# annalam/seqkit

Measured on AMD Instinct MI355X. Metric: M reads/s demultiplex (150bp, 96 barcodes) at 1/8 GPUs; % HBM roofline, higher is better.
Workload: dtype u8

## Files before the change

### seqkit_amd/csrc/sk_census.hip

```cpp
#include <hip/hip_runtime.h>

#include <algorithm>
#include <cstdlib>
#include <cstring>
#include <vector>

#include "sk_internal.h"

namespace sk {

typedef unsigned long long u64;
typedef uint32_t u32;

struct CensusSlot {
	u64 klo;
	u64 khi_inv;
	u64 count;
	u64 first_inv;
};

constexpr int kSpillBucketsLog2 = 8;
constexpr int kSpillBuckets = 1 << kSpillBucketsLog2;
__device__ __forceinline__ uint32_t census_bucket(uint32_t h) { return h >> (32 - kSpillBucketsLog2); }
constexpr int kSpillMaxLen = 24;
constexpr int kSpillMaxGrid = 1024;

struct CensusSpill {
	uint4 *key = nullptr;
	u32 *hist = nullptr;
	u32 *btot = nullptr;
	u32 *wg_count = nullptr;
	u32 *wg_stats = nullptr;
	u32 *work = nullptr;
	u32 cap = 0;
	u32 direct_above = 0;
	u32 grid = 0;
	u32 merge_copies = 0;
};

constexpr int kRecRowBits = 25;
__device__ __forceinline__ u32 census_rec_row(u32 w) { return w & ((1u << kRecRowBits) - 1u); }
__device__ __forceinline__ u32 census_rec_count(u32 w) { return (((w >> 27) & 31u) + 1u) << (5u * ((w >> kRecRowBits) & 3u)); }

struct Census {
	CensusSpill sp;
	size_t sp_records = 0;
	int sp_grid = 0;
	CensusSlot *tab = nullptr;
	u64 slots = 0;
	u32 *log = nullptr;
	u32 *log_count = nullptr;
	u32 log_cap = 0;
	u64 *stats = nullptr;
	u64 distinct = 0;
	u64 *scratch = nullptr;
	size_t scratch_bytes = 0;
};

constexpr int kCensusStats = 4;
constexpr u64 kInitialSlots = 1ull << 26;
constexpr u32 kLogCap = 1u << 16;
constexpr int64_t kCensusChunk = 1 << 25;
constexpr int64_t kCensusMinChunk = 1 << 22;
constexpr int kLdsSlots = 2048;
constexpr int kLdsProbes = 8;
constexpr u32 kMaxProbes = 1u << 16;

struct LdsTable {
	u64 klo[kLdsSlots];
	u64 khi_inv[kLdsSlots];
	u64 first_inv[kLdsSlots];
	u32 count[kLdsSlots];
};

__device__ __forceinline__ u32 census_hash(u64 klo, u64 khi)
{
	const u32 w0 = (u32)klo, w1 = (u32)(klo >> 32), w2 = (u32)khi, w3 = (u32)(khi >> 32);
	u32 h = w0 * 0x9E3779B1u ^ __builtin_rotateleft32(w1, 13) * 0x85EBCA77u ^ w2 * 0xC2B2AE3Du ^ __builtin_rotateleft32(w3, 7) * 0x27D4EB2Fu;
	h ^= h >> 15;
	h *= 0x2C1B3C6Du;
	h ^= h >> 12;
	h *= 0x297A2D39u;
	h ^= h >> 15;
	return h;
}

constexpr u32 kClassLo = 0x412B4300u;
constexpr u32 kClassHi = 0xFF54474Eu;
__device__ __forceinline__ u32 census_classify(u32 x, u32 &diff)
{
	const u32 lower = x & (x >> 1) & 0x20202020u;
	const u32 y = x ^ lower;
	const u32 sel = (y ^ (y >> 5)) & 0x07070707u;
	diff = y ^ __builtin_amdgcn_perm(kClassHi, kClassLo, sel);
	return sel | (lower >> 2);
}
static const char kCensusAlphabet[17] = "\0C+ANGT??c?angt?";

struct SlotView { u64 k, v; };

__device__ __forceinline__ SlotView census_peek(const CensusSlot *s)
{
	typedef u32 u32x4_t __attribute__((ext_vector_type(4)));
	u32x4_t w;
	asm volatile("global_load_dwordx4 %0, %1, off sc1" : "=&v"(w) : "v"(s) : "memory");
	__builtin_amdgcn_s_waitcnt(0x0F70);
	asm volatile("" : "+v"(w));
	SlotView sv;
	sv.k = (u64)w[0] | ((u64)w[1] << 32);
	sv.v = (u64)w[2] | ((u64)w[3] << 32);
	return sv;
}

constexpr int kLogRegions = 256;
struct CensusTab {
	CensusSlot *tab;
	u64 mask;
	u32 sh;
	u32 *log;
	u32 *log_count;
	u32 log_cap;
};

__device__ __forceinline__ void census_log_claim(const CensusTab &t, const CensusSlot *s)
{
	if (t.log_cap == 0u) return;
	const u64 m = __ballot(1);
	const int leader = __ffsll((unsigned long long)m) - 1;
	const u32 rank = __builtin_amdgcn_mbcnt_hi((u32)(m >> 32), __builtin_amdgcn_mbcnt_lo((u32)m, 0u));
// ... 694 lines not shown
		counted += __shfl_xor(counted, o);
		rejected += __shfl_xor(rejected, o);
		overflow += __shfl_xor(overflow, o);
	}
	__syncthreads();
	u32 *wg_stats = front;
	if (tid < kCensusStats) wg_stats[tid] = 0u;
	__syncthreads();
	if (lane == 0) {
		if (claimed) atomicAdd(&wg_stats[0], claimed);
		if (counted) atomicAdd(&wg_stats[1], counted);
		if (rejected) atomicAdd(&wg_stats[2], rejected);
		if (overflow) atomicAdd(&wg_stats[3], overflow);
	}
	__syncthreads();
	if (SPILL) { if (tid < kCensusStats) a.sp.wg_stats[blockIdx.x * kCensusStats + tid] = wg_stats[tid]; }
	else if (tid < kCensusStats && wg_stats[tid] != 0u) atomicAdd(&a.stats[tid], (u64)wg_stats[tid]);
#ifdef SK_CENSUS_STAMPS
	SK_STAMP(9);
	if (lane == 0 && blockIdx.x * nwave + wave < 8192)
		for (int i = 0; i < kStampSlots; i++) g_census_stamps[(blockIdx.x * nwave + wave) * kStampSlots + i] = st_acc[i];
#endif
}

__device__ __forceinline__ u32 census_block_exclusive(u32 mine, u32 *ws, u32 *total)
{
	const int lane = threadIdx.x & 63, wave = threadIdx.x >> 6, nw = (blockDim.x + 63) >> 6;
	u32 v = mine;
#pragma unroll
	for (int o = 1; o < 64; o <<= 1) {
		const u32 t = __shfl_up(v, o);
		if (lane >= o) v += t;
	}
	__syncthreads();
	if (lane == 63) ws[wave] = v;
	__syncthreads();
	if (wave == 0) {
		const u32 w = lane < nw ? ws[lane] : 0u;
		u32 x = w;
#pragma unroll
		for (int o = 1; o < 16; o <<= 1) {
			const u32 t = __shfl_up(x, o);
			if (lane >= o) x += t;
		}
		if (lane < nw) ws[lane] = x - w;
		if (lane == nw - 1) ws[16] = x;
	}
	__syncthreads();
	if (total) *total = ws[16];
	return v - mine + ws[wave];
}

__device__ __forceinline__ u32 census_spill_total(const CensusSpill &sp, u32 *red)
{
	u32 v = 0u;
	for (u32 g = threadIdx.x; g < sp.grid; g += blockDim.x) v += sp.wg_count[g];
	for (int o = 32; o > 0; o >>= 1) v += __shfl_xor(v, o);
	if ((threadIdx.x & 63) == 0) red[threadIdx.x >> 6] = v;
	__syncthreads();
	u32 tot = 0u;
	for (u32 w = 0; w < (blockDim.x + 63) / 64; w++) tot += red[w];
	__syncthreads();
	return tot;
}

__device__ __forceinline__ void census_add_stats(u64 *stats, u32 claimed, u32 overflow, u32 *red)
{
	for (int o = 32; o > 0; o >>= 1) {
		claimed += __shfl_xor(claimed, o);
		overflow += __shfl_xor(overflow, o);
	}
	__syncthreads();
	if (threadIdx.x < 2) red[threadIdx.x] = 0u;
	__syncthreads();
	if ((threadIdx.x & 63) == 0) {
		if (claimed) atomicAdd(&red[0], claimed);
		if (overflow) atomicAdd(&red[1], overflow);
	}
	__syncthreads();
	if (threadIdx.x == 0 && red[0] != 0u) atomicAdd(&stats[0], (u64)red[0]);
	if (threadIdx.x == 1 && red[1] != 0u) atomicAdd(&stats[3], (u64)red[1]);
}

constexpr int kCombineThreads = 512;
#ifndef SK_COMBINE_CHUNK
#define SK_COMBINE_CHUNK 16384
#endif
constexpr int kCombineChunk = SK_COMBINE_CHUNK;
__global__ __launch_bounds__(kCombineThreads, 4) void census_combine_kernel(const CensusArgs a)
{
	__shared__ LdsTable lt_s;
	__shared__ u32 cpre[kSpillBuckets + 1];
	__shared__ u32 gpre[kSpillMaxGrid + 1];
	__shared__ u32 red[kCombineThreads / 64];
	__shared__ u32 ws[17];
	__shared__ u32 item_s, nlist;
	__shared__ uint16_t list[kLdsSlots];
	LdsTable *lt = &lt_s;
	const int tid = threadIdx.x;
	const u32 grid = a.sp.grid;
#ifdef SK_CENSUS_STAMPS
	u64 cst_acc[kStampSlots] = {};
	u64 cst_last = __builtin_amdgcn_s_memtime();
#endif
	if (blockIdx.x == 0) {
		__shared__ u32 ssum[kCensusStats];
		if (tid < kCensusStats) ssum[tid] = 0u;
		__syncthreads();
		u32 v = 0u;
		for (u32 i = tid; i < grid * kCensusStats; i += blockDim.x) v += a.sp.wg_stats[i];
		for (int o = 32; o >= kCensusStats; o >>= 1) v += __shfl_xor(v, o);
		if ((tid & 63) < kCensusStats && v != 0u) atomicAdd(&ssum[tid & 3], v);
		__syncthreads();
		if (tid < kCensusStats && ssum[tid] != 0u) atomicAdd(&a.stats[tid], (u64)ssum[tid]);
	}
	if (census_spill_total(a.sp, red) > a.sp.direct_above) return;
	{
		static_assert(kSpillBuckets <= kCombineThreads, "one bucket per thread");
		const u32 c = tid < kSpillBuckets ? (a.sp.btot[tid] + kCombineChunk - 1) / kCombineChunk : 0u;
		u32 total;
		const u32 before = census_block_exclusive(c, ws, &total);
		if (tid < kSpillBuckets) cpre[tid] = before;
		if (tid == 0) cpre[kSpillBuckets] = total;
		__syncthreads();
	}
	const u32 items = cpre[kSpillBuckets];
	SK_CSTAMP(0);
	u32 claimed = 0, overflow = 0;
	int b_have = -1;
	for (;;) {
		__syncthreads();
		if (tid == 0) item_s = atomicAdd(a.sp.work, 1u);
		for (int i = tid; i < (int)(sizeof(LdsTable) / 8); i += blockDim.x) reinterpret_cast<u64 *>(lt)[i] = 0ull;
		__syncthreads();
		const u32 item = item_s;
		SK_CSTAMP(1);
		if (item >= items) break;
		int b = 0;
		for (int o = kSpillBuckets / 2; o > 0; o >>= 1) if (cpre[b + o] <= item) b += o;
		if (b != b_have) {
			u32 carry = 0u;
			for (u32 g0 = 0; g0 < grid; g0 += blockDim.x) {
				const u32 g = g0 + tid;
				const u32 v = g < grid ? a.sp.hist[(size_t)b * grid + g] : 0u;
				u32 total;
				const u32 before = census_block_exclusive(v, ws, &total);
				if (g < grid) gpre[g] = carry + before;
				carry += total;
			}
			if (tid == 0) gpre[grid] = carry;
			__syncthreads();
			b_have = b;
		}
		const u32 lo = (item - cpre[b]) * kCombineChunk;
		const u32 hi = min(gpre[grid], lo + kCombineChunk);
		u32 gcur = 0u;
		{
			const u32 i = lo + tid;
			u32 l = 0u, r = grid;
			while (r - l > 1u) { const u32 m = (l + r) >> 1; if (gpre[m] <= i) l = m; else r = m; }
			gcur = l;
		}
		SK_CSTAMP(2);
		const uint4 *const base = a.sp.key + (size_t)b * a.sp.cap;
		const size_t gpitch = (size_t)kSpillBuckets * a.sp.cap;
		constexpr int kAhead = 4;
		uint4 kk[kAhead], kn[kAhead];
		auto fetch = [&](u32 i0, uint4 (&dst)[kAhead]) {
#pragma unroll
			for (int q = 0; q < kAhead; q++) {
				const u32 i = i0 + (u32)q * blockDim.x;
				if (i < hi) {
					while (gpre[gcur + 1] <= i) gcur++;
					dst[q] = base[(size_t)gcur * gpitch + (i - gpre[gcur])];
				} else dst[q] = make_uint4(0u, 0u, 0u, 0u);
			}
		};
		fetch(lo + tid, kk);
		for (u32 i0 = lo + tid; i0 < hi; i0 += kAhead * blockDim.x) {
			fetch(i0 + kAhead * blockDim.x, kn);
			bool dir[kAhead], have[kAhead];
			u64 klo[kAhead], khi[kAhead], first_inv[kAhead];
			u32 cnt[kAhead], hh[kAhead];
#pragma unroll
			for (int q = 0; q < kAhead; q++) {
				const uint4 k = kk[q];
				have[q] = i0 + (u32)q * blockDim.x < hi;
				klo[q] = 0xF0000000ull | ((u64)k.x << 32);
				khi[q] = (u64)k.y | ((u64)k.z << 32);
				first_inv[q] = ~(u64)(a.row_base + census_rec_row(k.w));
				cnt[q] = census_rec_count(k.w);
				hh[q] = census_hash(klo[q], khi[q]);
			}
			SK_CSTAMP(3);
			lds_count_many<kAhead>(lt, have, hh, klo, khi, cnt, first_inv, dir);
			SK_CSTAMP(4);
			bool any_dir = false;
#pragma unroll
			for (int q = 0; q < kAhead; q++) any_dir = any_dir || dir[q];
			if (__any(any_dir)) census_insert_many<kAhead>(a.t, dir, klo, khi, cnt, first_inv, claimed, overflow);
			SK_CSTAMP(5);
#pragma unroll
			for (int q = 0; q < kAhead; q++) kk[q] = kn[q];
		}
		__syncthreads();
		SK_CSTAMP(6);
		if (tid == 0) nlist = 0u;
		__syncthreads();
		for (int i = tid; i < kLdsSlots; i += blockDim.x)
			if (lt->klo[i] != 0) list[atomicAdd(&nlist, 1u)] = (uint16_t)i;
		__syncthreads();
		for (u32 j0 = tid; j0 < nlist; j0 += kAhead * blockDim.x) {
			bool want[kAhead];
			u64 klo[kAhead], khi[kAhead], first_inv[kAhead];
			u32 cnt[kAhead];
#pragma unroll
			for (int q = 0; q < kAhead; q++) {
				const u32 j = j0 + (u32)q * blockDim.x;
				want[q] = j < nlist;
				const int i = list[want[q] ? j : 0u];
				klo[q] = lt->klo[i]; khi[q] = ~lt->khi_inv[i]; first_inv[q] = lt->first_inv[i]; cnt[q] = lt->count[i];
			}
			census_insert_many<kAhead>(a.t, want, klo, khi, cnt, first_inv, claimed, overflow);
		}
		SK_CSTAMP(7);
	}
	census_add_stats(a.stats, claimed, overflow, red);
#ifdef SK_CENSUS_STAMPS
	SK_CSTAMP(8);
	if ((tid & 63) == 0 && blockIdx.x * (kCombineThreads / 64) + (tid >> 6) < 8192)
		for (int i = 0; i < kStampSlots; i++) g_combine_stamps[(blockIdx.x * (kCombineThreads / 64) + (tid >> 6)) * kStampSlots + i] = cst_acc[i];
#endif
}

constexpr int kDirectThreads = 512;
__global__ __launch_bounds__(kDirectThreads) void census_direct_kernel(const CensusArgs a, const int split)
{
	__shared__ u32 red[16];
	const bool mine = census_spill_total(a.sp, red) > a.sp.direct_above;
	if (blockIdx.x == 0) {
		if (threadIdx.x < (u32)kSpillBuckets) a.sp.btot[threadIdx.x] = 0u;
		if (threadIdx.x == 0) *a.sp.work = 0u;
	}
	if (!mine) return;
	const u32 g = blockIdx.x / (u32)split, part = blockIdx.x % (u32)split;
	u32 claimed = 0, overflow = 0;
	__shared__ u32 bpre[kSpillBuckets + 1];
	__shared__ u32 ws[17];
	{
		static_assert(kSpillBuckets <= kDirectThreads, "one bucket per thread");
		const u32 v = threadIdx.x < (u32)kSpillBuckets ? a.sp.hist[(size_t)threadIdx.x * a.sp.grid + g] : 0u;
		u32 total;
		const u32 before = census_block_exclusive(v, ws, &total);
		if (threadIdx.x < (u32)kSpillBuckets) bpre[threadIdx.x] = before;
		if (threadIdx.x == 0) bpre[kSpillBuckets] = total;
		__syncthreads();
	}
	const u32 n = bpre[kSpillBuckets];
	const u32 rot = n != 0u ? (u32)(((u64)g * 0x9E3779B1ull) % n) : 0u;
	const uint4 *const key = a.sp.key + (size_t)g * kSpillBuckets * a.sp.cap;
	for (u32 jj = part * blockDim.x + threadIdx.x; jj < n; jj += (u32)split * blockDim.x) {
		u32 j = jj + rot;
		j = j >= n ? j - n : j;
		u32 l = 0u, r = (u32)kSpillBuckets;
		while (r - l > 1u) { const u32 m = (l + r) >> 1; if (bpre[m] <= j) l = m; else r = m; }
		const uint4 k = key[(size_t)l * a.sp.cap + (j - bpre[l])];
		const u64 klo = 0xF0000000ull | ((u64)k.x << 32), khi = (u64)k.y | ((u64)k.z << 32);
		const u32 c = census_rec_count(k.w);
		if (!census_insert(a.t, klo, khi, (u64)c, ~(u64)(a.row_base + census_rec_row(k.w)), claimed)) overflow += c;
	}
	census_add_stats(a.stats, claimed, overflow, red);
}

__global__ __launch_bounds__(256) void census_rehash_kernel(const CensusSlot *old_tab, u64 old_slots, const CensusTab t, u64 *stats)
{
	u32 claimed = 0, overflow = 0;
	for (u64 i = (u64)blockIdx.x * blockDim.x + threadIdx.x; i < old_slots; i += (u64)gridDim.x * blockDim.x) {
		const CensusSlot s = old_tab[i];
		if (s.klo == 0) continue;
		if (!census_insert(t, s.klo, ~s.khi_inv, s.count, s.first_inv, claimed)) overflow++;
	}
	if (overflow) atomicAdd(&stats[3], (u64)overflow);
}

__global__ __launch_bounds__(256) void census_hist_kernel(const CensusSlot *tab, u64 slots, u64 *hist)
{
	__shared__ u32 lh[64];
	if (threadIdx.x < 64) lh[threadIdx.x] = 0;
	__syncthreads();
	for (u64 i = (u64)blockIdx.x * blockDim.x + threadIdx.x; i < slots; i += (u64)gridDim.x * blockDim.x) {
		const u64 klo = tab[i].klo, c = tab[i].count;
		if (klo != 0 && c != 0) atomicAdd(&lh[63 - __clzll(c)], 1u);
	}
	__syncthreads();
	if (threadIdx.x < 64 && lh[threadIdx.x]) atomicAdd(&hist[threadIdx.x], (u64)lh[threadIdx.x]);
}

__global__ __launch_bounds__(256) void census_compact_kernel(const CensusSlot *tab, u64 slots, u64 min_count, u64 *out, u64 cap)
{
	for (u64 i = (u64)blockIdx.x * blockDim.x + threadIdx.x; i < slots; i += (u64)gridDim.x * blockDim.x) {
		const CensusSlot s = tab[i];
		if (s.klo != 0 && s.count >= min_count && s.count != 0) {
			const u64 at = atomicAdd(&out[0], 1ull);
			if (at < cap) {
				u64 *e = out + 4 + at * 4;
				e[0] = s.klo; e[1] = s.khi_inv; e[2] = s.count; e[3] = s.first_inv;
			}
		}
	}
}

constexpr int kCensusVariants = kCensusMaxSub * 3 * 2;
static const void *census_variant(int v)
{
// ... 61 lines not shown
	while ((1ull << lg) < cs->slots) lg++;
	t.sh = (u32)(32 - lg);
	t.log = cs->log;
	t.log_count = cs->log_count;
	t.log_cap = cs->log_cap;
	return t;
}

__global__ __launch_bounds__(256) void census_clear_kernel(const CensusTab t)
{
	__shared__ u32 cnt[kLogRegions];
	__shared__ u32 over;
	if (threadIdx.x == 0) over = 0u;
	__syncthreads();
	for (int r = threadIdx.x; r < kLogRegions; r += blockDim.x) {
		const u32 c = t.log_count[r * 32];
		cnt[r] = c < t.log_cap ? c : t.log_cap;
		if (c > t.log_cap || t.log_cap == 0u) over = 1u;
	}
	__syncthreads();
	uint4 *const p = reinterpret_cast<uint4 *>(t.tab);
	if (over) {
		const u64 n = (t.mask + 1) * (sizeof(CensusSlot) / 16);
		for (u64 i = (u64)blockIdx.x * blockDim.x + threadIdx.x; i < n; i += (u64)gridDim.x * blockDim.x) p[i] = make_uint4(0u, 0u, 0u, 0u);
		return;
	}
	const int r = blockIdx.x & (kLogRegions - 1);
	const u32 per = gridDim.x / kLogRegions ? gridDim.x / kLogRegions : 1u, part = blockIdx.x / kLogRegions;
	for (u32 i = part * blockDim.x + threadIdx.x; i < cnt[r]; i += per * blockDim.x) {
		const u64 slot = t.log[(size_t)r * t.log_cap + i];
		p[2 * slot] = make_uint4(0u, 0u, 0u, 0u);
		p[2 * slot + 1] = make_uint4(0u, 0u, 0u, 0u);
	}
}

hipError_t census_reset(Census *cs, int n_cu, hipStream_t st)
{
	hipError_t e = hipMemsetAsync(cs->stats, 0, kCensusStats * sizeof(u64), st);
	if (e == hipSuccess) {
		census_clear_kernel<<<kLogRegions * 8, 256, 0, st>>>(census_tab_of(cs));
		e = hipGetLastError();
	}
	if (e == hipSuccess) e = hipMemsetAsync(cs->log_count, 0, (size_t)kLogRegions * 32 * sizeof(u32), st);
	(void)n_cu;
	cs->distinct = 0;
	return e;
}

hipError_t census_stats(Census *cs, uint64_t out[4], hipStream_t st)
{
	u64 h[kCensusStats];
	hipError_t e = hipMemcpyAsync(h, cs->stats, sizeof h, hipMemcpyDeviceToHost, st);
	if (e == hipSuccess) e = hipStreamSynchronize(st);
	if (e != hipSuccess) return e;
	cs->distinct = h[0];
	for (int i = 0; i < kCensusStats; i++) out[i] = h[i];
	return hipSuccess;
}

uint64_t census_slots(const Census *cs) { return cs->slots; }

static hipError_t census_reserve(Census *cs, u64 incoming, int n_cu, hipStream_t st)
{
	const u64 need = 2 * (cs->distinct + incoming);
	if (need <= cs->slots) return hipSuccess;
	u64 slots = cs->slots;
	while (slots < need) slots <<= 1;
	if (slots > (1ull << 32)) return hipErrorOutOfMemory;
	CensusSlot *old_tab = cs->tab;
	const u64 old_slots = cs->slots;
	hipError_t e = census_alloc_table(cs, slots, st);
	if (e != hipSuccess) { (void)hipGetLastError(); cs->tab = old_tab; cs->slots = old_slots; return e; }
	e = hipMemsetAsync(cs->log_count, 0, (size_t)kLogRegions * 32 * sizeof(u32), st);
	if (e != hipSuccess) return e;
	census_rehash_kernel<<<n_cu * 8, 256, 0, st>>>(old_tab, old_slots, census_tab_of(cs), cs->stats);
	e = hipGetLastError();
	if (e == hipSuccess) e = hipStreamSynchronize(st);
	(void)hipFree(old_tab);
	return e;
}

static void census_spill_free(Census *cs)
{
	void *ptrs[] = {cs->sp.key, cs->sp.hist, cs->sp.btot, cs->sp.wg_count, cs->sp.wg_stats, cs->sp.work};
	for (void *q : ptrs) if (q) (void)hipFree(q);
	cs->sp = CensusSpill();
	cs->sp_records = 0;
	cs->sp_grid = 0;
}

static hipError_t census_spill_reserve(Census *cs, int grid, u32 cap, hipStream_t st)
{
	const size_t records = (size_t)grid * kSpillBuckets * cap;
	if (records <= cs->sp_records && grid <= cs->sp_grid) return hipSuccess;
	const size_t want_records = std::max(records, cs->sp_records);
	const int want_grid = std::max(grid, cs->sp_grid);
	hipError_t e = hipStreamSynchronize(st);
	if (e != hipSuccess) return e;
	census_spill_free(cs);
	e = hipMalloc((void **)&cs->sp.key, want_records * sizeof(uint4));
	if (e == hipSuccess) e = hipMalloc((void **)&cs->sp.hist, (size_t)want_grid * kSpillBuckets * sizeof(u32));
	if (e == hipSuccess) e = hipMalloc((void **)&cs->sp.btot, kSpillBuckets * sizeof(u32));
	if (e == hipSuccess) e = hipMalloc((void **)&cs->sp.wg_count, (size_t)want_grid * sizeof(u32));
	if (e == hipSuccess) e = hipMalloc((void **)&cs->sp.wg_stats, (size_t)want_grid * kCensusStats * sizeof(u32));
	if (e == hipSuccess) e = hipMalloc((void **)&cs->sp.work, sizeof(u32));
	if (e == hipSuccess) e = hipMemsetAsync(cs->sp.btot, 0, kSpillBuckets * sizeof(u32), st);
	if (e == hipSuccess) e = hipMemsetAsync(cs->sp.work, 0, sizeof(u32), st);
	if (e != hipSuccess) { (void)hipGetLastError(); census_spill_free(cs); return e; }
	cs->sp_records = want_records;
	cs->sp_grid = want_grid;
	return hipSuccess;
}

constexpr int64_t kSpillMinRows = 1 << 19;

hipError_t census_add(Census *cs, const uint8_t *bc, int bc_stride, int L, int64_t n, const int32_t *assign, int64_t row_base,
                      int n_cu, hipStream_t st)
{
	if (bc_stride > kCensusMaxStride) return hipErrorInvalidValue;
	int R = kCensusStepBytes / (64 * bc_stride);
	R = R < 1 ? 1 : (R > kCensusMaxSub ? kCensusMaxSub : R);
	if (const char *ev = getenv("SK_CENSUS_TILES")) { const int v = atoi(ev); if (v >= 1 && v <= R) R = v; }
	const int nw_dwords = L <= 8 ? 2 : (L <= 20 ? 5 : 8);
	auto slot_bytes = [&](int r, bool spill_layout) {
		const int queue_cap = 64 + r * 64;
		int bytes = queue_cap * (4 * nw_dwords + 4);
		if (!spill_layout) {
			const int flush_end = ((queue_cap * 4 + 64 * 4 * nw_dwords + 15) & ~15) + kCensusQueue * 20;
			if (bytes < flush_end) bytes = flush_end;
		}
		return (bytes + 15) & ~15;
	};
	const int nw_class = L <= 8 ? 0 : (L <= 20 ? 1 : 2);
	const int front_entry_bytes = nw_class == 2 ? 52 : 36;
	auto plan_lds = [&](int r, bool spill_layout, int &tile_slot, int &front_entries) {
		tile_slot = slot_bytes(r, spill_layout);
		size_t lds = (size_t)kCensusWaves * tile_slot + 64 + (kSpillBuckets + 4) * sizeof(u32);
		front_entries = (int)((160 * 1024 - 16 - lds) / front_entry_bytes) & ~63;
		if (const char *ev = getenv("SK_CENSUS_FRONT_ENTRIES")) { const int v = atoi(ev) & ~63; if (v >= 64 && v <= front_entries) front_entries = v; }
		return lds + (((size_t)front_entries * front_entry_bytes + 15) & ~(size_t)15);
	};
	int wgs_per_cu = 1;
	if (const char *ev = getenv("SK_CENSUS_WGS")) { const int v = atoi(ev); if (v >= 1 && v <= 4) wgs_per_cu = v; }
	int direct_pct = 50;
	if (const char *ev = getenv("SK_CENSUS_SPILL_MAX_PCT")) { const int v = atoi(ev); if (v >= 0 && v <= 100) direct_pct = v; }
	int64_t spill_min_rows = kSpillMinRows;
	if (const char *ev = getenv("SK_CENSUS_SPILL_MIN_ROWS_LOG2")) { const int lg = atoi(ev); if (lg >= 6 && lg <= 30) spill_min_rows = (int64_t)1 << lg; }
	int direct_split = 8;
	if (const char *ev = getenv("SK_CENSUS_DIRECT_SPLIT")) { const int v = atoi(ev); if (v >= 1 && v <= 64) direct_split = v; }
	int merge_copies = 1;
	if (const char *ev = getenv("SK_CENSUS_MERGE_RECORDS")) merge_copies = atoi(ev) != 0;
	int spill_mode = -1;
	if (const char *ev = getenv("SK_CENSUS_SPILL")) spill_mode = atoi(ev) != 0;
	int64_t chunk = kCensusChunk, min_chunk = kCensusMinChunk;
	if (const char *ev = getenv("SK_CENSUS_CHUNK_LOG2")) { const int lg = atoi(ev); if (lg >= 6 && lg <= kRecRowBits) chunk = (int64_t)1 << lg; }
	if (const char *ev = getenv("SK_CENSUS_MIN_CHUNK_LOG2")) { const int lg = atoi(ev); if (lg >= 6 && lg <= 30) min_chunk = (int64_t)1 << lg; }
	{
		const int64_t max_rows = ((((int64_t)1 << 31) - (1 << 24)) / bc_stride) & ~(int64_t)63;
		if (chunk > max_rows) chunk = max_rows;
	}
	if (min_chunk > chunk) min_chunk = chunk;
	int64_t nr = 0;
	for (int64_t o = 0; o < n; o += nr) {
		nr = (n - o) < chunk ? (n - o) : chunk;
		hipError_t e = hipSuccess;
		if (2 * (cs->distinct + (u64)nr) > cs->slots && !getenv("SK_CENSUS_TRUST_SLOTS")) {
			uint64_t s[4];
			e = census_stats(cs, s, st);
			if (e != hipSuccess) return e;
			const int64_t room = (int64_t)(cs->slots / 2) - (int64_t)cs->distinct;
			const int64_t least = nr < min_chunk ? nr : min_chunk;
			if (room >= least) nr = nr < room ? nr : room;
			else e = census_reserve(cs, (u64)nr, n_cu, st);
			if (e != hipSuccess) return e;
			if (nr < n - o && nr >= 64) nr &= ~(int64_t)63;
		}
		cs->distinct += (u64)nr;
		CensusArgs a;
		a.bc = bc + o * (int64_t)bc_stride;
		a.bc_stride = bc_stride;
		a.L = L;
		a.n = nr;
		a.assign = assign ? assign + o : nullptr;
		a.row_base = row_base + o;
		a.t = census_tab_of(cs);
		a.stats = cs->stats;
		a.long_way_only = getenv("SK_CENSUS_LONG_WAY_ONLY") && atoi(getenv("SK_CENSUS_LONG_WAY_ONLY")) != 0;
		bool spill = L <= kSpillMaxLen && (spill_mode < 0 ? nr >= spill_min_rows : spill_mode != 0);
		const int Rk = (spill && nw_class >= 1 && !getenv("SK_CENSUS_TILES")) ? 1 : R;
		auto grid_of = [&](int r) {
			const int64_t groups = (nr + (int64_t)64 * r * kCensusWaves - 1) / ((int64_t)64 * r * kCensusWaves);
			const int g = n_cu * wgs_per_cu;
			return g > groups ? (int)groups : g;
		};
		int grid = grid_of(Rk);
		a.sp = CensusSpill();
		if (spill) {
			const int64_t nsteps = (nr + (int64_t)64 * Rk - 1) / ((int64_t)64 * Rk);
			const int64_t per_wave = (nsteps + (int64_t)grid * kCensusWaves - 1) / ((int64_t)grid * kCensusWaves);
			const int64_t wg_rows = per_wave * kCensusWaves * Rk * 64;
			const int64_t cap = (((wg_rows + kSpillBuckets - 1) / kSpillBuckets) * 2 + 256 + 7) & ~(int64_t)7;
			e = (grid <= kSpillMaxGrid && cap * kSpillBuckets < ((int64_t)1 << 27)) ? census_spill_reserve(cs, grid, (u32)cap, st) : hipErrorInvalidValue;
			if (e != hipSuccess) { (void)hipGetLastError(); spill = false; grid = grid_of(Rk); }
			else {
				a.sp = cs->sp;
				a.sp.cap = (u32)cap;
				a.sp.grid = (u32)grid;
				a.sp.direct_above = (u32)((uint64_t)nr * (uint64_t)direct_pct / 100);
				a.sp.merge_copies = (u32)merge_copies;
			}
		}
		int tile_slot = 0, front_entries = 0;
		const size_t lds = plan_lds(Rk, spill, tile_slot, front_entries);
		hipLaunchKernelGGL(reinterpret_cast<void (*)(const CensusArgs, const int, const int)>(const_cast<void *>(census_variant(((Rk - 1) * 3 + nw_class) * 2 + (spill ? 1 : 0)))),
		                   dim3(grid), dim3(kCensusWaves * 64), lds, st, a, tile_slot, front_entries);
		if (spill) {
			census_combine_kernel<<<2 * n_cu, kCombineThreads, 0, st>>>(a);
			census_direct_kernel<<<grid * direct_split, kDirectThreads, 0, st>>>(a, direct_split);
		}
		e = hipGetLastError();
		if (e != hipSuccess) return e;
	}
	return hipSuccess;
}

static hipError_t census_scratch(Census *cs, size_t bytes)
{
	if (bytes <= cs->scratch_bytes) return hipSuccess;
	if (cs->scratch) { (void)hipFree(cs->scratch); cs->scratch = nullptr; cs->scratch_bytes = 0; }
	hipError_t e = hipMalloc((void **)&cs->scratch, bytes);
	if (e == hipSuccess) cs->scratch_bytes = bytes;
	return e;
}

hipError_t census_count_hist(Census *cs, uint64_t hist[64], int n_cu, hipStream_t st)
{
	hipError_t e = census_scratch(cs, 64 * sizeof(u64));
	if (e == hipSuccess) e = hipMemsetAsync(cs->scratch, 0, 64 * sizeof(u64), st);
	if (e != hipSuccess) return e;
	census_hist_kernel<<<n_cu * 8, 256, 0, st>>>(cs->tab, cs->slots, cs->scratch);
	e = hipGetLastError();
	if (e == hipSuccess) e = hipMemcpyAsync(hist, cs->scratch, 64 * sizeof(u64), hipMemcpyDeviceToHost, st);
	if (e == hipSuccess) e = hipStreamSynchronize(st);
	return e;
}

hipError_t census_entries(Census *cs, uint64_t min_count, CensusEntry *out, uint64_t cap, uint64_t *total, int n_cu, hipStream_t st)
{
	uint64_t s[4];
	hipError_t e = census_stats(cs, s, st);
	if (e != hipSuccess) return e;
	const u64 room = std::min<u64>(cap, s[0]);
	e = census_scratch(cs, (4 + room * 4) * sizeof(u64));
	if (e == hipSuccess) e = hipMemsetAsync(cs->scratch, 0, 4 * sizeof(u64), st);
	if (e != hipSuccess) return e;
	census_compact_kernel<<<n_cu * 8, 256, 0, st>>>(cs->tab, cs->slots, min_count ? min_count : 1, cs->scratch, room);
	e = hipGetLastError();
	if (e != hipSuccess) return e;
	u64 found = 0;
	e = hipMemcpyAsync(&found, cs->scratch, sizeof found, hipMemcpyDeviceToHost, st);
	if (e == hipSuccess) e = hipStreamSynchronize(st);
	if (e != hipSuccess) return e;
	*total = found;
	const u64 got = std::min<u64>(found, room);
	std::vector<u64> raw(got * 4);
	if (got) {
		e = hipMemcpy(raw.data(), cs->scratch + 4, got * 4 * sizeof(u64), hipMemcpyDeviceToHost);
		if (e != hipSuccess) return e;
	}
	std::vector<u64> order(got);
	for (u64 i = 0; i < got; i++) order[i] = i;
	std::sort(order.begin(), order.end(), [&](u64 x, u64 y) { return raw[x * 4 + 3] > raw[y * 4 + 3]; });
	for (u64 i = 0; i < got; i++) {
		const u64 *r = &raw[order[i] * 4];
		const u64 klo = r[0], khi = ~r[1];
		const u32 kw[4] = {(u32)(klo >> 32), (u32)khi, (u32)(khi >> 32), (u32)klo};
		CensusEntry &en = out[i];
		memset(en.barcode, 0, sizeof en.barcode);
		for (int j = 0; j < 31; j++) {
			const int q = j >> 2, b = j & 3;
			const u32 c = (kw[q >> 1] >> (8 * b + 4 * (q & 1))) & 15u;
			if (c == 0) break;
			en.barcode[j] = kCensusAlphabet[c];
		}
		en.count = r[2];
		en.first_row = (int64_t)~r[3];
	}
	return hipSuccess;
}

}

#ifdef SK_CENSUS_STAMPS
extern "C" int sk_debug_census_stamps(unsigned long long *out, int waves)
{
	return (int)hipMemcpyFromSymbol(out, HIP_SYMBOL(sk::g_census_stamps), (size_t)waves * sk::kStampSlots * sizeof(unsigned long long));
}
extern "C" int sk_debug_combine_stamps(unsigned long long *out, int waves)
{
// ... 4 lines not shown
```

Before: 6767.

## Sub-partition large spill buckets by hash before combine for LDS locality

Adds two passes, subcount and subscatter, that split each large spill bucket into up to 512 hash sub-buckets and scatter the records into a contiguous sub-key buffer. The combine kernel then handles each sub-bucket range as one work item, so each workgroup's LDS table sees a narrower key range and fewer keys fall through to direct global-table inserts. Work items are also claimed in batches of four to reduce contention on the shared work counter. The cost is two extra kernel launches, an extra read and write of the spilled records, and a larger scratch allocation.

```diff
diff --git a/seqkit_amd/csrc/sk_census.hip b/seqkit_amd/csrc/sk_census.hip
--- a/seqkit_amd/csrc/sk_census.hip
+++ b/seqkit_amd/csrc/sk_census.hip
@@ -36,7 +36,17 @@
 	u32 direct_above = 0;
 	u32 grid = 0;
 	u32 merge_copies = 0;
+	uint4 *skey = nullptr;
+	u32 *subcnt = nullptr;
+	u32 *subcur = nullptr;
+	u32 *subpre = nullptr;
+	u32 *subitems = nullptr;
+	u32 sub_cap = 0;
+	u32 sub_above = 0;
+	u32 sub_split = 0;
 };
+constexpr int kSubMaxLog2 = 9;
+constexpr int kSubMax = 1 << kSubMaxLog2;
 
 constexpr int kRecRowBits = 25;
 __device__ __forceinline__ u32 census_rec_row(u32 w) { return w & ((1u << kRecRowBits) - 1u); }
@@ -45,6 +55,7 @@
 struct Census {
 	CensusSpill sp;
 	size_t sp_records = 0;
+	size_t sp_sub_records = 0;
 	int sp_grid = 0;
 	CensusSlot *tab = nullptr;
 	u64 slots = 0;
@@ -905,7 +916,210 @@
 	if (threadIdx.x == 1 && red[1] != 0u) atomicAdd(&stats[3], (u64)red[1]);
 }
 
+constexpr u32 kSubTarget = 1024;
+constexpr u32 kSubAbove = 4096;
+constexpr u32 kSubSplit = 4096;
 constexpr int kCombineThreads = 512;
+constexpr int kPartAhead = 4;
+constexpr u32 kPartChunk = kPartAhead * kCombineThreads;
+
+__device__ __forceinline__ int census_sub_log2(const CensusSpill &sp, u32 n)
+{
+	if (n <= sp.sub_above) return 0;
+	const u32 target = min(kSubTarget, max(sp.sub_above, 1u));
+	const u32 want = (n + target - 1u) / target;
+	const int lg = 32 - __clz((int)(want - 1u));
+	return lg > kSubMaxLog2 ? kSubMaxLog2 : lg;
+}
+__device__ __forceinline__ u32 census_sub_of(u32 h, int lg) { return (h >> (32 - kSpillBucketsLog2 - lg)) & ((1u << lg) - 1u); }
+__device__ __forceinline__ u32 census_rec_hash(const uint4 k) { return census_hash(0xF0000000ull | ((u64)k.x << 32), (u64)k.y | ((u64)k.z << 32)); }
+
+__device__ __forceinline__ void census_scan_regions(const CensusSpill &sp, int b, u32 *gpre, u32 *ws)
+{
+	const u32 grid = sp.grid;
+	u32 carry = 0u;
+	for (u32 g0 = 0; g0 < grid; g0 += blockDim.x) {
+		const u32 g = g0 + threadIdx.x;
+		const u32 v = g < grid ? sp.hist[(size_t)b * grid + g] : 0u;
+		u32 total;
+		const u32 before = census_block_exclusive(v, ws, &total);
+		if (g < grid) gpre[g] = carry + before;
+		carry += total;
+	}
+	if (threadIdx.x == 0) gpre[grid] = carry;
+	__syncthreads();
+}
+__device__ __forceinline__ u32 census_region_of(const u32 *gpre, u32 grid, u32 i)
+{
+	u32 l = 0u, r = grid;
+	while (r - l > 1u) { const u32 m = (l + r) >> 1; if (gpre[m] <= i) l = m; else r = m; }
+	return l;
+}
+__device__ __forceinline__ uint4 census_region_record(const CensusSpill &sp, int b, const u32 *gpre, u32 &gcur, u32 i)
+{
+	while (gpre[gcur + 1] <= i) gcur++;
+	return sp.key[(size_t)b * sp.cap + (size_t)gcur * kSpillBuckets * sp.cap + (i - gpre[gcur])];
+}
+
+__device__ __forceinline__ bool census_part_plan(const CensusSpill &sp, u32 *cpre, u32 *bbase, uint8_t *blg, u32 *red, u32 *ws)
+{
+	static_assert(kSpillBuckets <= kCombineThreads, "one bucket per thread");
+	if (census_spill_total(sp, red) > sp.direct_above) return false;
+	const int tid = threadIdx.x;
+	const u32 bt = tid < kSpillBuckets ? sp.btot[tid] : 0u;
+	const int lg = tid < kSpillBuckets ? census_sub_log2(sp, bt) : 0;
+	u32 total;
+	u32 before = census_block_exclusive(lg ? (bt + kPartChunk - 1u) / kPartChunk : 0u, ws, &total);
+	if (tid < kSpillBuckets) { cpre[tid] = before; blg[tid] = (uint8_t)lg; }
+	if (tid == 0) cpre[kSpillBuckets] = total;
+	if (bbase) {
+		before = census_block_exclusive(lg ? bt : 0u, ws, nullptr);
+		if (tid < kSpillBuckets) bbase[tid] = before;
+	}
+	__syncthreads();
+	return cpre[kSpillBuckets] != 0u;
+}
+
+#ifdef SK_CENSUS_STAMPS
+#define SK_PART_STAMPS_BEGIN u64 cst_acc[kStampSlots] = {}; u64 cst_last = __builtin_amdgcn_s_memtime()
+#define SK_PART_STAMPS_END(first, n) do { if ((threadIdx.x & 63) == 0 && blockIdx.x * (kCombineThreads / 64) + (threadIdx.x >> 6) < 8192) \
+		for (int i_ = (first); i_ < (first) + (n); i_++) g_combine_stamps[(blockIdx.x * (kCombineThreads / 64) + (threadIdx.x >> 6)) * kStampSlots + i_] = cst_acc[i_]; } while (0)
+#else
+#define SK_PART_STAMPS_BEGIN do { } while (0)
+#define SK_PART_STAMPS_END(first, n) do { } while (0)
+#endif
+
+__global__ __launch_bounds__(kCombineThreads) void census_subcount_kernel(const CensusArgs a)
+{
+	__shared__ u32 cpre[kSpillBuckets + 1];
+	__shared__ u32 gpre[kSpillMaxGrid + 1];
+	__shared__ u32 cnt[kSubMax];
+	__shared__ u32 red[kCombineThreads / 64];
+	__shared__ u32 ws[17];
+	__shared__ uint8_t blg[kSpillBuckets];
+	const int tid = threadIdx.x;
+	SK_PART_STAMPS_BEGIN;
+	if (!census_part_plan(a.sp, cpre, nullptr, blg, red, ws)) { SK_PART_STAMPS_END(9, 2); return; }
+	const u32 chunks = cpre[kSpillBuckets];
+	const u32 c0 = (u32)((u64)blockIdx.x * chunks / gridDim.x), c1 = (u32)((u64)(blockIdx.x + 1u) * chunks / gridDim.x);
+	SK_CSTAMP(9);
+	int b_have = -1, lg = 0;
+	auto flush = [&]() {
+		__syncthreads();
+		if (b_have >= 0)
+			for (u32 s = tid; s < (1u << lg); s += blockDim.x)
+				if (cnt[s] != 0u) atomicAdd(&a.sp.subcnt[(size_t)b_have * kSubMax + s], cnt[s]);
+		__syncthreads();
+	};
+	for (u32 c = c0; c < c1; c++) {
+		int b = 0;
+		for (int o = kSpillBuckets / 2; o > 0; o >>= 1) if (cpre[b + o] <= c) b += o;
+		if (b != b_have) {
+			flush();
+			census_scan_regions(a.sp, b, gpre, ws);
+			lg = blg[b];
+			for (u32 s = tid; s < (1u << lg); s += blockDim.x) cnt[s] = 0u;
+			__syncthreads();
+			b_have = b;
+		}
+		const u32 lo = (c - cpre[b]) * kPartChunk;
+		const u32 hi = min(gpre[a.sp.grid], lo + kPartChunk);
+		u32 gcur = census_region_of(gpre, a.sp.grid, lo + tid);
+		uint4 k[kPartAhead];
+#pragma unroll
+		for (int q = 0; q < kPartAhead; q++) {
+			const u32 i = lo + tid + (u32)q * blockDim.x;
+			k[q] = i < hi ? census_region_record(a.sp, b, gpre, gcur, i) : make_uint4(0u, 0u, 0u, 0u);
+		}
+#pragma unroll
+		for (int q = 0; q < kPartAhead; q++)
+			if (lo + tid + (u32)q * blockDim.x < hi) atomicAdd(&cnt[census_sub_of(census_rec_hash(k[q]), lg)], 1u);
+	}
+	flush();
+	SK_CSTAMP(10);
+	SK_PART_STAMPS_END(9, 2);
+}
+
+__global__ __launch_bounds__(kCombineThreads) void census_subscatter_kernel(const CensusArgs a)
+{
+	__shared__ u32 cpre[kSpillBuckets + 1];
+	__shared__ u32 bbase[kSpillBuckets];
+	__shared__ u32 gpre[kSpillMaxGrid + 1];
+	__shared__ u32 cnt[kSubMax];
+	__shared__ u32 spre[kSubMax];
+	__shared__ u32 red[kCombineThreads / 64];
+	__shared__ u32 ws[17];
+	__shared__ uint8_t blg[kSpillBuckets];
+	static_assert(kSubMax <= kCombineThreads, "one sub-bucket per thread");
+	const int tid = threadIdx.x;
+	SK_PART_STAMPS_BEGIN;
+	if (!census_part_plan(a.sp, cpre, bbase, blg, red, ws)) { SK_PART_STAMPS_END(11, 4); return; }
+	const u32 chunks = cpre[kSpillBuckets];
+	const u32 split = max(a.sp.sub_split, 1u);
+	for (u32 b = blockIdx.x; b < (u32)kSpillBuckets; b += gridDim.x) {
+		const int lgb = blg[b];
+		if (lgb == 0) continue;
+		const u32 nsub = 1u << lgb;
+		const u32 v = (u32)tid < nsub ? a.sp.subcnt[(size_t)b * kSubMax + tid] : 0u;
+		u32 total;
+		u32 before = census_block_exclusive(v, ws, &total);
+		if ((u32)tid < nsub) a.sp.subpre[(size_t)b * (kSubMax + 1) + tid] = bbase[b] + before;
+		if (tid == 0) a.sp.subpre[(size_t)b * (kSubMax + 1) + nsub] = bbase[b] + total;
+		before = census_block_exclusive((v + split - 1u) / split, ws, &total);
+		if ((u32)tid < nsub) a.sp.subitems[(size_t)b * (kSubMax + 1) + tid] = before;
+		if (tid == 0) a.sp.subitems[(size_t)b * (kSubMax + 1) + nsub] = total;
+	}
+	const u32 c0 = (u32)((u64)blockIdx.x * chunks / gridDim.x), c1 = (u32)((u64)(blockIdx.x + 1u) * chunks / gridDim.x);
+	SK_CSTAMP(11);
+	int b_have = -1, lg = 0;
+	for (u32 c = c0; c < c1; c++) {
+		int b = 0;
+		for (int o = kSpillBuckets / 2; o > 0; o >>= 1) if (cpre[b + o] <= c) b += o;
+		__syncthreads();
+		if (b != b_have) {
+			census_scan_regions(a.sp, b, gpre, ws);
+			lg = blg[b];
+			const u32 v = (u32)tid < (1u << lg) ? a.sp.subcnt[(size_t)b * kSubMax + tid] : 0u;
+			const u32 before = census_block_exclusive(v, ws, nullptr);
+			if ((u32)tid < (1u << lg)) spre[tid] = bbase[b] + before;
+			b_have = b;
+		}
+		for (u32 s = tid; s < (1u << lg); s += blockDim.x) cnt[s] = 0u;
+		__syncthreads();
+		const u32 lo = (c - cpre[b]) * kPartChunk;
+		const u32 hi = min(gpre[a.sp.grid], lo + kPartChunk);
+		u32 gcur = census_region_of(gpre, a.sp.grid, lo + tid);
+		uint4 k[kPartAhead];
+		u32 sub[kPartAhead], rank[kPartAhead];
+#pragma unroll
+		for (int q = 0; q < kPartAhead; q++) {
+			const u32 i = lo + tid + (u32)q * blockDim.x;
+			k[q] = i < hi ? census_region_record(a.sp, b, gpre, gcur, i) : make_uint4(0u, 0u, 0u, 0u);
+		}
+#pragma unroll
+		for (int q = 0; q < kPartAhead; q++) {
+			sub[q] = census_sub_of(census_rec_hash(k[q]), lg);
+			rank[q] = 0u;
+			if (lo + tid + (u32)q * blockDim.x < hi) rank[q] = atomicAdd(&cnt[sub[q]], 1u);
+		}
+		__syncthreads();
+		SK_CSTAMP(12);
+		for (u32 s = tid; s < (1u << lg); s += blockDim.x) {
+			const u32 n = cnt[s];
+			cnt[s] = spre[s] + (n != 0u ? atomicAdd(&a.sp.subcur[(size_t)b * kSubMax + s], n) : 0u);
+		}
+		__syncthreads();
+		SK_CSTAMP(13);
+#pragma unroll
+		for (int q = 0; q < kPartAhead; q++) {
+			const u32 at = cnt[sub[q]] + rank[q];
+			if (lo + tid + (u32)q * blockDim.x < hi && at < a.sp.sub_cap) a.sp.skey[at] = k[q];
+		}
+		SK_CSTAMP(14);
+	}
+	SK_PART_STAMPS_END(11, 4);
+}
+
 #ifndef SK_COMBINE_CHUNK
 #define SK_COMBINE_CHUNK 16384
 #endif
@@ -915,16 +1129,21 @@
 	__shared__ LdsTable lt_s;
 	__shared__ u32 cpre[kSpillBuckets + 1];
 	__shared__ u32 gpre[kSpillMaxGrid + 1];
+	__shared__ u32 sipre[kSubMax + 1];
+	__shared__ u32 sspre[kSubMax + 1];
 	__shared__ u32 red[kCombineThreads / 64];
 	__shared__ u32 ws[17];
 	__shared__ u32 item_s, nlist;
+	__shared__ u32 drawn[2];
 	__shared__ uint16_t list[kLdsSlots];
+	__shared__ uint8_t blg[kSpillBuckets];
 	LdsTable *lt = &lt_s;
 	const int tid = threadIdx.x;
 	const u32 grid = a.sp.grid;
 #ifdef SK_CENSUS_STAMPS
 	u64 cst_acc[kStampSlots] = {};
 	u64 cst_last = __builtin_amdgcn_s_memtime();
+	u32 hbm_ops = 0u;
 #endif
 	if (blockIdx.x == 0) {
 		__shared__ u32 ssum[kCensusStats];
@@ -940,20 +1159,30 @@
 	if (census_spill_total(a.sp, red) > a.sp.direct_above) return;
 	{
 		static_assert(kSpillBuckets <= kCombineThreads, "one bucket per thread");
-		const u32 c = tid < kSpillBuckets ? (a.sp.btot[tid] + kCombineChunk - 1) / kCombineChunk : 0u;
+		const u32 bt = tid < kSpillBuckets ? a.sp.btot[tid] : 0u;
+		const int lg = tid < kSpillBuckets ? census_sub_log2(a.sp, bt) : 0;
+		const u32 c = lg ? a.sp.subitems[(size_t)tid * (kSubMax + 1) + (1u << lg)] : (bt + kCombineChunk - 1) / kCombineChunk;
 		u32 total;
 		const u32 before = census_block_exclusive(c, ws, &total);
-		if (tid < kSpillBuckets) cpre[tid] = before;
+		if (tid < kSpillBuckets) { cpre[tid] = before; blg[tid] = (uint8_t)lg; }
 		if (tid == 0) cpre[kSpillBuckets] = total;
 		__syncthreads();
 	}
+	for (u32 b = blockIdx.x; b < (u32)kSpillBuckets; b += gridDim.x)
+		for (u32 s = tid; blg[b] != 0 && s < (1u << blg[b]); s += blockDim.x) { a.sp.subcnt[(size_t)b * kSubMax + s] = 0u; a.sp.subcur[(size_t)b * kSubMax + s] = 0u; }
 	const u32 items = cpre[kSpillBuckets];
+	const u32 batch = items >= 8u * gridDim.x ? 4u : 1u;
+	const u32 split = max(a.sp.sub_split, 1u);
 	SK_CSTAMP(0);
 	u32 claimed = 0, overflow = 0;
-	int b_have = -1;
+	if (tid == 0) drawn[0] = drawn[1] = 0u;
+	int b_have = -1, sb_have = -1;
 	for (;;) {
 		__syncthreads();
-		if (tid == 0) item_s = atomicAdd(a.sp.work, 1u);
+		if (tid == 0) {
+			if (drawn[0] == drawn[1]) { drawn[0] = atomicAdd(a.sp.work, batch); drawn[1] = drawn[0] + batch; }
+			item_s = drawn[0]++;
+		}
 		for (int i = tid; i < (int)(sizeof(LdsTable) / 8); i += blockDim.x) reinterpret_cast<u64 *>(lt)[i] = 0ull;
 		__syncthreads();
 		const u32 item = item_s;
@@ -961,42 +1190,41 @@
 		if (item >= items) break;
 		int b = 0;
 		for (int o = kSpillBuckets / 2; o > 0; o >>= 1) if (cpre[b + o] <= item) b += o;
-		if (b != b_have) {
-			u32 carry = 0u;
-			for (u32 g0 = 0; g0 < grid; g0 += blockDim.x) {
-				const u32 g = g0 + tid;
-				const u32 v = g < grid ? a.sp.hist[(size_t)b * grid + g] : 0u;
-				u32 total;
-				const u32 before = census_block_exclusive(v, ws, &total);
-				if (g < grid) gpre[g] = carry + before;
-				carry += total;
-			}
-			if (tid == 0) gpre[grid] = carry;
-			__syncthreads();
-			b_have = b;
-		}
-		const u32 lo = (item - cpre[b]) * kCombineChunk;
-		const u32 hi = min(gpre[grid], lo + kCombineChunk);
-		u32 gcur = 0u;
-		{
-			const u32 i = lo + tid;
-			u32 l = 0u, r = grid;
-			while (r - l > 1u) { const u32 m = (l + r) >> 1; if (gpre[m] <= i) l = m; else r = m; }
-			gcur = l;
-		}
+		const bool lin = blg[b] != 0;
+		u32 lo, hi;
+		if (lin) {
+			const u32 nsub = 1u << blg[b];
+			if (b != sb_have) {
+				for (u32 s = tid; s <= nsub; s += blockDim.x) {
+					sipre[s] = a.sp.subitems[(size_t)b * (kSubMax + 1) + s];
+					sspre[s] = a.sp.subpre[(size_t)b * (kSubMax + 1) + s];
+				}
+				__syncthreads();
+				sb_have = b;
+			}
+			const u32 li = item - cpre[b];
+			u32 s = 0u;
+			for (u32 o = nsub >> 1; o > 0u; o >>= 1) if (sipre[s + o] <= li) s += o;
+			lo = sspre[s] + (li - sipre[s]) * split;
+			hi = min(min(sspre[s + 1], lo + split), a.sp.sub_cap);
+		} else {
+			if (b != b_have) {
+				census_scan_regions(a.sp, b, gpre, ws);
+				b_have = b;
+			}
+			lo = (item - cpre[b]) * kCombineChunk;
+			hi = min(gpre[grid], lo + kCombineChunk);
+		}
+		u32 gcur = lin ? 0u : census_region_of(gpre, grid, lo + tid);
 		SK_CSTAMP(2);
-		const uint4 *const base = a.sp.key + (size_t)b * a.sp.cap;
-		const size_t gpitch = (size_t)kSpillBuckets * a.sp.cap;
 		constexpr int kAhead = 4;
 		uint4 kk[kAhead], kn[kAhead];
 		auto fetch = [&](u32 i0, uint4 (&dst)[kAhead]) {
 #pragma unroll
 			for (int q = 0; q < kAhead; q++) {
 				const u32 i = i0 + (u32)q * blockDim.x;
-				if (i < hi) {
-					while (gpre[gcur + 1] <= i) gcur++;
-					dst[q] = base[(size_t)gcur * gpitch + (i - gpre[gcur])];
-				} else dst[q] = make_uint4(0u, 0u, 0u, 0u);
+				if (i < hi) dst[q] = lin ? a.sp.skey[i] : census_region_record(a.sp, b, gpre, gcur, i);
+				else dst[q] = make_uint4(0u, 0u, 0u, 0u);
 			}
 		};
 		fetch(lo + tid, kk);
@@ -1021,6 +1249,10 @@
 			bool any_dir = false;
 #pragma unroll
 			for (int q = 0; q < kAhead; q++) any_dir = any_dir || dir[q];
+#ifdef SK_CENSUS_STAMPS
+#pragma unroll
+			for (int q = 0; q < kAhead; q++) hbm_ops += dir[q] ? 1u : 0u;
+#endif
 			if (__any(any_dir)) census_insert_many<kAhead>(a.t, dir, klo, khi, cnt, first_inv, claimed, overflow);
 			SK_CSTAMP(5);
 #pragma unroll
@@ -1043,6 +1275,9 @@
 				want[q] = j < nlist;
 				const int i = list[want[q] ? j : 0u];
 				klo[q] = lt->klo[i]; khi[q] = ~lt->khi_inv[i]; first_inv[q] = lt->first_inv[i]; cnt[q] = lt->count[i];
+#ifdef SK_CENSUS_STAMPS
+				hbm_ops += want[q] ? 1u : 0u;
+#endif
 			}
 			census_insert_many<kAhead>(a.t, want, klo, khi, cnt, first_inv, claimed, overflow);
 		}
@@ -1051,8 +1286,11 @@
 	census_add_stats(a.stats, claimed, overflow, red);
 #ifdef SK_CENSUS_STAMPS
 	SK_CSTAMP(8);
+	for (int o = 32; o > 0; o >>= 1) hbm_ops += __shfl_xor(hbm_ops, o);
+	cst_acc[kStampSlots - 1] = hbm_ops;
 	if ((tid & 63) == 0 && blockIdx.x * (kCombineThreads / 64) + (tid >> 6) < 8192)
-		for (int i = 0; i < kStampSlots; i++) g_combine_stamps[(blockIdx.x * (kCombineThreads / 64) + (tid >> 6)) * kStampSlots + i] = cst_acc[i];
+		for (int i = 0; i < kStampSlots; i++)
+			if (i < 9 || i == kStampSlots - 1) g_combine_stamps[(blockIdx.x * (kCombineThreads / 64) + (tid >> 6)) * kStampSlots + i] = cst_acc[i];
 #endif
 }
 
@@ -1280,18 +1518,20 @@
 
 static void census_spill_free(Census *cs)
 {
-	void *ptrs[] = {cs->sp.key, cs->sp.hist, cs->sp.btot, cs->sp.wg_count, cs->sp.wg_stats, cs->sp.work};
+	void *ptrs[] = {cs->sp.key, cs->sp.hist, cs->sp.btot, cs->sp.wg_count, cs->sp.wg_stats, cs->sp.work, cs->sp.skey, cs->sp.subcnt};
 	for (void *q : ptrs) if (q) (void)hipFree(q);
 	cs->sp = CensusSpill();
 	cs->sp_records = 0;
+	cs->sp_sub_records = 0;
 	cs->sp_grid = 0;
 }
 
-static hipError_t census_spill_reserve(Census *cs, int grid, u32 cap, hipStream_t st)
+static hipError_t census_spill_reserve(Census *cs, int grid, u32 cap, size_t sub_records, hipStream_t st)
 {
 	const size_t records = (size_t)grid * kSpillBuckets * cap;
-	if (records <= cs->sp_records && grid <= cs->sp_grid) return hipSuccess;
+	if (records <= cs->sp_records && grid <= cs->sp_grid && sub_records <= cs->sp_sub_records) return hipSuccess;
 	const size_t want_records = std::max(records, cs->sp_records);
+	const size_t want_sub = std::max(std::max(sub_records, cs->sp_sub_records), (size_t)1);
 	const int want_grid = std::max(grid, cs->sp_grid);
 	hipError_t e = hipStreamSynchronize(st);
 	if (e != hipSuccess) return e;
@@ -1302,10 +1542,20 @@
 	if (e == hipSuccess) e = hipMalloc((void **)&cs->sp.wg_count, (size_t)want_grid * sizeof(u32));
 	if (e == hipSuccess) e = hipMalloc((void **)&cs->sp.wg_stats, (size_t)want_grid * kCensusStats * sizeof(u32));
 	if (e == hipSuccess) e = hipMalloc((void **)&cs->sp.work, sizeof(u32));
+	if (e == hipSuccess) e = hipMalloc((void **)&cs->sp.skey, want_sub * sizeof(uint4));
+	const size_t sub_words = (size_t)kSpillBuckets * (2 * kSubMax + 2 * (kSubMax + 1));
+	if (e == hipSuccess) e = hipMalloc((void **)&cs->sp.subcnt, sub_words * sizeof(u32));
+	if (e == hipSuccess) {
+		cs->sp.subcur = cs->sp.subcnt + (size_t)kSpillBuckets * kSubMax;
+		cs->sp.subpre = cs->sp.subcur + (size_t)kSpillBuckets * kSubMax;
+		cs->sp.subitems = cs->sp.subpre + (size_t)kSpillBuckets * (kSubMax + 1);
+		e = hipMemsetAsync(cs->sp.subcnt, 0, sub_words * sizeof(u32), st);
+	}
 	if (e == hipSuccess) e = hipMemsetAsync(cs->sp.btot, 0, kSpillBuckets * sizeof(u32), st);
 	if (e == hipSuccess) e = hipMemsetAsync(cs->sp.work, 0, sizeof(u32), st);
 	if (e != hipSuccess) { (void)hipGetLastError(); census_spill_free(cs); return e; }
 	cs->sp_records = want_records;
+	cs->sp_sub_records = want_sub;
 	cs->sp_grid = want_grid;
 	return hipSuccess;
 }
@@ -1348,6 +1598,9 @@
 	if (const char *ev = getenv("SK_CENSUS_DIRECT_SPLIT")) { const int v = atoi(ev); if (v >= 1 && v <= 64) direct_split = v; }
 	int merge_copies = 1;
 	if (const char *ev = getenv("SK_CENSUS_MERGE_RECORDS")) merge_copies = atoi(ev) != 0;
+	u32 sub_above = kSubAbove, sub_split = kSubSplit;
+	if (const char *ev = getenv("SK_CENSUS_SUB_MIN_RECORDS_LOG2")) { const int lg = atoi(ev); if (lg >= 4 && lg <= 30) sub_above = 1u << lg; }
+	if (const char *ev = getenv("SK_CENSUS_SUB_SPLIT_LOG2")) { const int lg = atoi(ev); if (lg >= 4 && lg <= 24) sub_split = 1u << lg; }
 	int spill_mode = -1;
 	if (const char *ev = getenv("SK_CENSUS_SPILL")) spill_mode = atoi(ev) != 0;
 	int64_t chunk = kCensusChunk, min_chunk = kCensusMinChunk;
@@ -1398,14 +1651,18 @@
 			const int64_t per_wave = (nsteps + (int64_t)grid * kCensusWaves - 1) / ((int64_t)grid * kCensusWaves);
 			const int64_t wg_rows = per_wave * kCensusWaves * Rk * 64;
 			const int64_t cap = (((wg_rows + kSpillBuckets - 1) / kSpillBuckets) * 2 + 256 + 7) & ~(int64_t)7;
-			e = (grid <= kSpillMaxGrid && cap * kSpillBuckets < ((int64_t)1 << 27)) ? census_spill_reserve(cs, grid, (u32)cap, st) : hipErrorInvalidValue;
+			const uint64_t direct_above = (uint64_t)nr * (uint64_t)direct_pct / 100;
+			e = (grid <= kSpillMaxGrid && cap * kSpillBuckets < ((int64_t)1 << 27)) ? census_spill_reserve(cs, grid, (u32)cap, (size_t)direct_above, st) : hipErrorInvalidValue;
 			if (e != hipSuccess) { (void)hipGetLastError(); spill = false; grid = grid_of(Rk); }
 			else {
 				a.sp = cs->sp;
 				a.sp.cap = (u32)cap;
 				a.sp.grid = (u32)grid;
-				a.sp.direct_above = (u32)((uint64_t)nr * (uint64_t)direct_pct / 100);
+				a.sp.direct_above = (u32)direct_above;
 				a.sp.merge_copies = (u32)merge_copies;
+				a.sp.sub_cap = (u32)cs->sp_sub_records;
+				a.sp.sub_above = sub_above;
+				a.sp.sub_split = sub_split;
 			}
 		}
 		int tile_slot = 0, front_entries = 0;
@@ -1413,6 +1670,8 @@
 		hipLaunchKernelGGL(reinterpret_cast<void (*)(const CensusArgs, const int, const int)>(const_cast<void *>(census_variant(((Rk - 1) * 3 + nw_class) * 2 + (spill ? 1 : 0)))),
 		                   dim3(grid), dim3(kCensusWaves * 64), lds, st, a, tile_slot, front_entries);
 		if (spill) {
+			census_subcount_kernel<<<2 * n_cu, kCombineThreads, 0, st>>>(a);
+			census_subscatter_kernel<<<2 * n_cu, kCombineThreads, 0, st>>>(a);
 			census_combine_kernel<<<2 * n_cu, kCombineThreads, 0, st>>>(a);
 			census_direct_kernel<<<grid * direct_split, kDirectThreads, 0, st>>>(a, direct_split);
 		}
```

Result: slower. 6642 (-1.8%).
